# ZhenghaoFei/visual_odom

Hardware: AMD Instinct MI355X
Metric: stereo frames/sec on KITTI-00 1241x376 @ ~2000 features (higher is better)
Workload: dtype u8/int32 LK (f32 2x2 solve), f64 pose solve

## Files before the change

### visual_odom_amd/csrc/lk.hip

```cpp
#include "vo_kernels.h"
#include "vo_lkmath.h"

#include <float.h>
#include <type_traits>

namespace vo {

constexpr int LK_WIN = 21;
constexpr int LK_JT_W = 48, LK_JT_H = 40;
constexpr int LK_W_BITS = 14;
template <int W>
struct LkWin {
    static_assert(W % 2 == 1 && W >= 5 && W <= LK_WIN, "odd windows of 5 .. 21: the pyramid's borders are laid out for 21");
    static constexpr int SEGS = (W + 6) / 7, LANES = W * SEGS, COLS = 7 * SEGS + 1, ROWS = W + 1, LAST = W - 7 * (SEGS - 1);
    static constexpr int OFF_X = ((LK_JT_W - COLS) / 2) & ~3, OFF_Y = (LK_JT_H - ROWS) / 2;
    static_assert(LANES <= 64 && LK_JT_W >= COLS + OFF_X + 3 && LK_JT_H >= ROWS + OFF_Y, "the lane map and the tile hold the window");
};
constexpr uint32_t lk_seg_mask(int valid, int m)
{
    return (2 * m < valid ? 0x0000ffffu : 0u) | (2 * m + 1 < valid ? 0xffff0000u : 0u);
}

template <bool COLS>
__device__ __forceinline__ void lk_weights_packed(float a, float b, uint32_t &w0, uint32_t &w1)
{
    const float s = (float)(1 << LK_W_BITS), magic = 12582912.f;
    const float a1 = (1.f - a) * s, a0 = a * s, b1 = 1.f - b;
    const uint32_t r00 = (uint32_t)__float_as_int(a1 * b1 + magic);
    const uint32_t r01 = (uint32_t)__float_as_int(a0 * b1 + magic);
    const uint32_t r10 = (uint32_t)__float_as_int(a1 * b + magic);
    const uint32_t iw11 = ((1u << LK_W_BITS) + 3u * 0x4B400000u) - (r00 + r01 + r10);
    w0 = perm_b32(COLS ? r10 : r01, r00, VO_SEL_LO16);
    w1 = perm_b32(iw11, COLS ? r01 : r10, VO_SEL_LO16);
}
__device__ __forceinline__ void lk_weights(float a, float b, uint32_t &wt, uint32_t &wb)
{
    lk_weights_packed<false>(a, b, wt, wb);
}
__device__ __forceinline__ void lk_weights_cols(float a, float b, uint32_t &wl, uint32_t &wr)
{
    lk_weights_packed<true>(a, b, wl, wr);
}

struct LkOrigin {
    int x, y;
};
template <int W = LK_WIN>
__device__ __forceinline__ bool lk_tile_misses(bool have_tile, int jx0, int jy0, int inx, int iny)
{
    return !have_tile || inx < jx0 || inx + LkWin<W>::COLS > jx0 + LK_JT_W || iny < jy0 || iny + LkWin<W>::ROWS > jy0 + LK_JT_H;
}
template <int W = LK_WIN>
__device__ __forceinline__ LkOrigin lk_tile_origin(int jx_max, int jy_max, int inx, int iny)
{
    int jx0 = (inx - LkWin<W>::OFF_X) & ~3;
    int jy0 = iny - LkWin<W>::OFF_Y;
    jx0 = jx0 < -VO_BX ? -VO_BX : jx0 > jx_max ? jx_max : jx0;
    jy0 = jy0 < -VO_BY ? -VO_BY : jy0 > jy_max ? jy_max : jy0;
    return LkOrigin{jx0, jy0};
}
template <int W = LK_WIN>
__device__ __forceinline__ LkOrigin lk_tile_refill(uint8_t *tile, const VO_GLOBAL uint8_t *__restrict__ Jimg, int jstride, int jx_max, int jy_max,
                                               int inx, int iny, int c0, int step)
{
    const LkOrigin org = lk_tile_origin<W>(jx_max, jy_max, inx, iny);
    const int jx0 = org.x, jy0 = org.y;
    const VO_GLOBAL uint8_t *tb = Jimg + (ptrdiff_t)jy0 * jstride + jx0;
    for (int c = c0; c < LK_JT_H * (LK_JT_W / 16); c += step) {
        const int row = c / (LK_JT_W / 16), col = c - row * (LK_JT_W / 16);
        const U32x4A4 v = *(const VO_GLOBAL U32x4A4 *)(tb + (uint32_t)(row * jstride + 16 * col));
        *reinterpret_cast<uint4 *>(&tile[row * LK_JT_W + 16 * col]) = make_uint4(v.a, v.b, v.c, v.d);
    }
    return org;
}
template <int W = LK_WIN>
__device__ __forceinline__ LkOrigin lk_tile_refill_wave(uint8_t *tile, const VO_GLOBAL uint8_t *__restrict__ Jimg, int jstride, int jx_max,
                                                    int jy_max, int inx, int iny, int lane)
{
    constexpr int CPR = LK_JT_W / 16, CHUNKS = LK_JT_H * CPR;
    static_assert(CPR == 3 && CHUNKS > 64 && CHUNKS <= 128, "two chunks per lane at most; 64 chunks = 21 rows + 1 chunk");
    const LkOrigin org = lk_tile_origin<W>(jx_max, jy_max, inx, iny);
    const VO_GLOBAL uint8_t *tb = Jimg + (ptrdiff_t)org.y * jstride + org.x;
#ifndef VO_HOST_EMUL
    asm volatile("" : "+v"(lane));
#endif
    const int row = (lane * 43) >> 7, col = lane - CPR * row;
    const uint32_t g0 = (uint32_t)(row * jstride + 16 * col);
    const int next_col = 21 * jstride + 16, next_row = 22 * jstride - 16 * (CPR - 1);
    const uint32_t g1 = g0 + (uint32_t)(col == CPR - 1 ? next_row : next_col);
    const bool second = lane < CHUNKS - 64;
    const U32x4A4 v0 = *(const VO_GLOBAL U32x4A4 *)(tb + g0);
    U32x4A4 v1 = v0;
    if (second)
        v1 = *(const VO_GLOBAL U32x4A4 *)(tb + g1);
    *reinterpret_cast<uint4 *>(&tile[16 * lane]) = make_uint4(v0.a, v0.b, v0.c, v0.d);
    if (second)
        *reinterpret_cast<uint4 *>(&tile[16 * lane + 1024]) = make_uint4(v1.a, v1.b, v1.c, v1.d);
    return org;
}
template <int W = LK_WIN>
__device__ __forceinline__ LkOrigin lk_tile_cover(uint8_t *tile, const VO_GLOBAL uint8_t *__restrict__ Jimg, int jstride, int jx_max, int jy_max,
                                              int inx, int iny, int lane, bool have_tile, int jx0, int jy0)
{
    if (!lk_tile_misses<W>(have_tile, jx0, jy0, inx, iny))
        return LkOrigin{jx0, jy0};
    __syncthreads();
    const LkOrigin o = lk_tile_refill_wave<W>(tile, Jimg, jstride, jx_max, jy_max, inx, iny, lane);
    __syncthreads();
    return o;
}
__device__ __forceinline__ void lk_cell_rows(const uint8_t *tile, int off, uint32_t Jt[7], uint32_t Jb[7])
{
    const U32x2A1 t = *reinterpret_cast<const U32x2A1 *>(&tile[off]);
    const U32x2A1 u = *reinterpret_cast<const U32x2A1 *>(&tile[off + LK_JT_W]);
    lift7(t.a, t.b, Jt);
    lift7(u.a, u.b, Jb);
}
__device__ __forceinline__ void lk_cell_cols(const uint8_t *tile, int off, uint32_t Jc[8])
{
    const U32x2A1 t = *reinterpret_cast<const U32x2A1 *>(&tile[off]);
    const U32x2A1 u = *reinterpret_cast<const U32x2A1 *>(&tile[off + LK_JT_W]);
    lift8_cols(t.a, t.b, u.a, u.b, Jc);
}

#ifndef VO_LK_ATTRS
#define VO_LK_ATTRS __launch_bounds__(64, 7)
#endif
constexpr int VO_LK_USE_INITIAL_FLOW = 4, VO_LK_GET_MIN_EIGENVALS = 8;
template <bool SPLIT, bool ERR, int WIN = LK_WIN, bool FLAGS = false>
__device__ __forceinline__ void lk_circular_body(const PyrImage *__restrict__ imgs, const Quad *__restrict__ quads,
                                                 const float2 *__restrict__ pts_in, const int *__restrict__ n_pts, int cap,
                                                 int n_frames, int fpg , int ppp ,
                                                 float2 *__restrict__ trk,
                                                 uint8_t *__restrict__ status,
                                                 const LkParams prm, int hop_begin, int hop_end, float *__restrict__ err = nullptr,
                                                 int flags = 0)
{
    __shared__ __attribute__((aligned(16))) uint8_t s_jt[LK_JT_H * LK_JT_W];

    const int bid = blockIdx.x;
    const int xcd = bid & 7, slot = bid >> 3;
    const int grp = slot / ppp, fi = slot - grp * ppp;
    const int frame = grp * fpg + (xcd & (fpg - 1));
    const int f = (xcd / fpg) * ppp + fi;
    if (frame >= n_frames || f >= n_pts[frame])
        return;
    const int lane = threadIdx.x;
    using LW = LkWin<WIN>;
    const bool live = lane < LW::LANES;
    const int lr = live ? lane : LW::LANES - 1;
    const int r = lr / LW::SEGS, c0 = 7 * (lr - LW::SEGS * r);
    const int lane_off = r * LK_JT_W + c0;

    const Quad q = quads[frame];
    const float halfWin = (WIN - 1) * 0.5f;
    const float FLT_SCALE = 1.f / (1 << 20);
    const float eps_lo = (float)(prm.epsilon * 0.999999), eps_hi = (float)(prm.epsilon * 1.000001);
    const float min_eig_n = prm.min_eig * (1.001f * (float)(2 * WIN * WIN));

    const float2 p = pts_in[(size_t)frame * cap + f];
    float prevPtX = unif(p.x), prevPtY = unif(p.y);
    if (SPLIT && hop_begin > 0) {
        const size_t o = ((size_t)frame * 4 + (hop_begin - 1)) * cap + f;
        const float2 q0 = trk[o];
        const bool dead0 = status[o] == 0 || q0.x < 0.f || q0.y < 0.f || (hop_begin == 1 && (p.x < 0.f || p.y < 0.f));
        if (dead0 && !prm.full_chain)
            return;
        prevPtX = unif(q0.x);
        prevPtY = unif(q0.y);
    }

    for (int hop = SPLIT ? hop_begin : 0; hop < (ERR ? 1 : SPLIT ? hop_end : 4); hop++) {
        const int pi = hop == 0 ? q.l0 : hop == 1 ? q.r0 : hop == 2 ? q.r1 : q.l1;
        const int ni = hop == 0 ? q.r0 : hop == 1 ? q.r1 : hop == 2 ? q.l1 : q.l0;
        const PyrImage &I = imgs[pi];
        const PyrImage &J = imgs[ni];
        float outX = 0.f, outY = 0.f;
        int st = 1;
        float errv = 0.f;

        for (int level = prm.max_level; level >= 0; level--) {
            const float scale = __int_as_float((127 - level) << 23);
            float prevX = prevPtX * scale, prevY = prevPtY * scale;
            float nextX, nextY;
            if (level == prm.max_level) {
                nextX = prevX;
                nextY = prevY;
                if constexpr (FLAGS) {
                    if (flags & VO_LK_USE_INITIAL_FLOW) {
                        const float2 g = trk[(size_t)frame * cap + f];
                        nextX = unif(g.x) * scale;
                        nextY = unif(g.y) * scale;
                    }
                }
            } else {
                nextX = outX * 2.f;
                nextY = outY * 2.f;
            }
            outX = nextX;
            outY = nextY;

            const int iw = I.w[level], ih = I.h[level], istride = I.stride[level];
            const int jw = J.w[level], jh = J.h[level], jstride = J.stride[level];
            const VO_GLOBAL uint8_t *__restrict__ Iimg = (const VO_GLOBAL uint8_t *)I.lvl[level];
            const VO_GLOBAL uint32_t *__restrict__ Ider = (const VO_GLOBAL uint32_t *)I.der[level];
            const VO_GLOBAL uint8_t *__restrict__ Jimg = (const VO_GLOBAL uint8_t *)J.lvl[level];

            prevX -= halfWin;
            prevY -= halfWin;
            const float fpx = floorf(prevX), fpy = floorf(prevY);
            const int ipx = uni(vo_f2i(fpx)), ipy = uni(vo_f2i(fpy));
            if (VO_BALLOT(__builtin_isunordered(fpx, fpy)) != 0ull || ipx < -WIN || ipx >= iw || ipy < -WIN || ipy >= ih) {
                if (level == 0)
                    st = 0;
                continue;
            }
            uint32_t wl, wr;
            lk_weights_cols(prevX - fpx, prevY - fpy, wl, wr);

            uint32_t Ixp[4], Iyp[4];
            uint32_t Ipe[ERR ? 4 : 1];
            int a11 = 0, a12 = 0, a22 = 0, c1 = 0, c2 = 0;
            {
                const ptrdiff_t org = (ptrdiff_t)VO_BY * istride + VO_BX;
                const VO_GLOBAL uint8_t *Ib = Iimg - org;
                const VO_GLOBAL uint8_t *Db = (const VO_GLOBAL uint8_t *)(Ider - org);
                const uint32_t o = (uint32_t)((ipy + r + VO_BY) * istride + ipx + c0 + VO_BX);
                const uint32_t od = live ? 4u * o : 0u, drow = 4u * (uint32_t)istride;
                const U32x2A1 t = *(const VO_GLOBAL U32x2A1 *)(Ib + o);
                const U32x2A1 u = *(const VO_GLOBAL U32x2A1 *)(Ib + (o + (uint32_t)istride));
                const U32x4A4 dt0 = *(const VO_GLOBAL U32x4A4 *)(Db + od);
                const U32x4A4 dt1 = *(const VO_GLOBAL U32x4A4 *)(Db + (od + 16u));
                const U32x4A4 db0 = *(const VO_GLOBAL U32x4A4 *)(Db + (od + drow));
                const U32x4A4 db1 = *(const VO_GLOBAL U32x4A4 *)(Db + (od + drow + 16u));
                const uint32_t dt[8] = {dt0.a, dt0.b, dt0.c, dt0.d, dt1.a, dt1.b, dt1.c, dt1.d};
                const uint32_t db[8] = {db0.a, db0.b, db0.c, db0.d, db1.a, db1.b, db1.c, db1.d};
                uint32_t Ip[4];
                bilinear7_u8_cols(t.a, t.b, u.a, u.b, wl, wr, Ip);
                bilinear7_deriv_cols(dt, db, wl, wr, Ixp, Iyp);
                if constexpr (LW::LAST < 7) {
                    const bool part = LW::SEGS == 1 || c0 == 7 * (LW::SEGS - 1);
#pragma unroll
                    for (int m = 0; m < 4; m++) {
                        const uint32_t keep = part ? lk_seg_mask(LW::LAST, m) : 0xffffffffu;
                        Ixp[m] &= keep;
                        Iyp[m] &= keep;
                    }
                }
                a11 = sdot2_first(Ixp[0], Ixp[0], 0);
                a12 = sdot2_first(Ixp[0], Iyp[0], 0);
                a22 = sdot2_first(Iyp[0], Iyp[0], 0);
                c1 = sdot2_first(Ip[0], Ixp[0], 0);
                c2 = sdot2_first(Ip[0], Iyp[0], 0);
#pragma unroll
                for (int m = 1; m < 4; m++) {
                    a11 = sdot2(Ixp[m], Ixp[m], a11);
                    a12 = sdot2(Ixp[m], Iyp[m], a12);
                    a22 = sdot2(Iyp[m], Iyp[m], a22);
                    c1 = sdot2(Ip[m], Ixp[m], c1);
                    c2 = sdot2(Ip[m], Iyp[m], c2);
                }
                if constexpr (ERR) {
#pragma unroll
                    for (int m = 0; m < 4; m++)
                        Ipe[m] = Ip[m];
                }
            }
            float A11, A12, A22;
            wave_sum3_exact_f32(a11, a12, a22, A11, A12, A22);
            A11 *= FLT_SCALE;
            A12 *= FLT_SCALE;
            A22 *= FLT_SCALE;

            float D = A11 * A22 - A12 * A12;
            const float t = A22 + A11;
            const float s2 = (A11 - A22) * (A11 - A22) + 4.f * A12 * A12;
            const float u = t - (min_eig_n + t * 3.814697265625e-6f);
            bool eig_ok = u > 0.f && s2 < u * u * 0.9999f;
            if (__builtin_expect(!eig_ok, 0)) {
#ifndef VO_HOST_EMUL
                asm volatile("" ::: "memory");
#endif
                const float minEig = (t - sqrtf(s2)) / (float)(2 * WIN * WIN);
                eig_ok = !(minEig < prm.min_eig);
            }
            if constexpr (FLAGS) {
                if ((flags & VO_LK_GET_MIN_EIGENVALS) && level == 0)
                    errv = (t - sqrtf(s2)) / (float)(2 * WIN * WIN);
            }
            if (!eig_ok || D < FLT_EPSILON) {
                if (level == 0)
                    st = 0;
                continue;
            }
            D = 1.f / D;
            const float A11s = A11 * FLT_SCALE, A12s = A12 * FLT_SCALE, A22s = A22 * FLT_SCALE;
            const int nc1 = -c1, nc2 = -c2;

            nextX -= halfWin;
            nextY -= halfWin;
            float prevDX = 0.f, prevDY = 0.f;
            int jx0 = 0, jy0 = 0;
            bool have_tile = false;
            static_assert(LK_JT_W % 16 == 0 && VO_BX % 4 == 0, "16-byte tile chunks at 4-byte aligned origins");
            static_assert(VO_BY >= WIN && LK_JT_W >= LW::COLS + LW::OFF_X + 3 && LK_JT_H >= LW::ROWS + LW::OFF_Y,
                          "a tile clamped to the row end / the last border row still covers what the window of every corner the "
                          "reference admits reads (up to w - 1, h - 1: the borders are at least a window wide)");
            static_assert(VO_BY >= LW::COLS - 1, "right border (at least VO_BY columns) >= the columns a row reads beyond corner w - 1");
            const int jx_max = jstride - VO_BX - LK_JT_W, jy_max = jh + VO_BY - LK_JT_H;

            int j = 0;
            float fnx = floorf(nextX), fny = floorf(nextY);
            bool run = prm.max_count > 0;
            while (run) {
                const int inx = uni(vo_f2i(fnx)), iny = uni(vo_f2i(fny));
                if (VO_BALLOT(__builtin_isunordered(fnx, fny)) != 0ull || inx < -WIN || inx >= jw || iny < -WIN || iny >= jh) {
                    if (level == 0)
                        st = 0;
                    break;
                }
                {
                    const LkOrigin o = lk_tile_cover<WIN>(s_jt, Jimg, jstride, jx_max, jy_max, inx, iny, lane, have_tile, jx0, jy0);
                    jx0 = o.x;
                    jy0 = o.y;
                    have_tile = true;
                }
                uint32_t Jc[8];
                lk_cell_cols(s_jt, (iny - jy0) * LK_JT_W + (inx - jx0) + lane_off, Jc);
                for (;;) {
                    lk_weights_cols(nextX - fnx, nextY - fny, wl, wr);
                    int b1, b2;
                    {
                        uint32_t Jp[4];
                        blend7_cols(Jc, wl, wr, Jp);
                        b1 = sdot2_first(Jp[0], Ixp[0], nc1);
                        b2 = sdot2_first(Jp[0], Iyp[0], nc2);
#pragma unroll
                        for (int m = 1; m < 4; m++) {
                            b1 = sdot2(Jp[m], Ixp[m], b1);
                            b2 = sdot2(Jp[m], Iyp[m], b2);
                        }
                    }
                    float fb1, fb2;
                    wave_sum2_exact_f32(b1, b2, fb1, fb2);
                    const float dx = (A12s * fb2 - A22s * fb1) * D;
                    const float dy = (A12s * fb1 - A11s * fb2) * D;
                    nextX += dx;
                    nextY += dy;
                    outX = nextX + halfWin;
                    outY = nextY + halfWin;
                    const float n2 = fmaf(dy, dy, dx * dx);
                    if (__builtin_expect(!(n2 > eps_hi), 0)) {
#ifndef VO_HOST_EMUL
                        asm volatile("" ::: "memory");
#endif
                        if (n2 < eps_lo || (double)dx * dx + (double)dy * dy <= prm.epsilon) {
                            run = false;
                            break;
                        }
                    }
                    if (j > 0 && fabsf(dx + prevDX) <= 0.01f && fabsf(dy + prevDY) <= 0.01f) {
#ifndef VO_HOST_EMUL
                        asm volatile("" ::: "memory");
#endif
                        outX -= dx * 0.5f;
                        outY -= dy * 0.5f;
                        run = false;
                        break;
                    }
                    prevDX = dx;
                    prevDY = dy;
                    if (++j >= prm.max_count) {
                        run = false;
                        break;
                    }
                    const uint32_t ua = (uint32_t)__float_as_int(nextX - fnx), ub = (uint32_t)__float_as_int(nextY - fny);
                    if (VO_BALLOT((ua > ub ? ua : ub) >= 0x3f800000u) != 0ull) {
                        fnx = floorf(nextX);
                        fny = floorf(nextY);
                        break;
                    }
                }
            }

            if (st && level == 0 && (!FLAGS || !(flags & VO_LK_GET_MIN_EIGENVALS))) {
                const int fx = vo_f2i(floorf(outX - halfWin)), fy = vo_f2i(floorf(outY - halfWin));
                if (fx < -WIN || fx >= jw || fy < -WIN || fy >= jh)
                    st = 0;
                if constexpr (ERR) {
                    if (st && err != nullptr) {
                        const float ex = outX - halfWin, ey = outY - halfWin;
                        const float fex = floorf(ex), fey = floorf(ey);
                        const int inx = uni(fx), iny = uni(fy);
                        const LkOrigin o = lk_tile_cover<WIN>(s_jt, Jimg, jstride, jx_max, jy_max, inx, iny, lane, have_tile, jx0, jy0);
                        jx0 = o.x;
                        jy0 = o.y;
                        uint32_t Jc[8], Jp[4];
                        lk_cell_cols(s_jt, (iny - jy0) * LK_JT_W + (inx - jx0) + lane_off, Jc);
                        lk_weights_cols(ex - fex, ey - fey, wl, wr);
                        blend7_cols(Jc, wl, wr, Jp);
                        uint32_t e = 0;
#pragma unroll
                        for (int m = 0; m < 4; m++) {
                            if constexpr (LW::LAST < 7) {
                                const bool part = LW::SEGS == 1 || c0 == 7 * (LW::SEGS - 1);
                                e = udot2(pk_absdiff_i16(Jp[m], Ipe[m]) & (part ? lk_seg_mask(LW::LAST, m) : 0xffffffffu), 0x00010001u, e);
                            } else
                                e = udot2(pk_absdiff_i16(Jp[m], Ipe[m]), 0x00010001u, e);
                        }
                        errv = wave_sum_exact_f32(live ? (int)e : 0) / (float)(32 * WIN * WIN);
                    }
                }
            }
        }

        if constexpr (ERR) {
            if (lane == 0) {
                trk[(size_t)frame * cap + f] = make_float2(outX, outY);
                status[(size_t)frame * cap + f] = (uint8_t)st;
                if (err != nullptr) {
                    if constexpr (FLAGS)
                        err[(size_t)frame * cap + f] = ((flags & VO_LK_GET_MIN_EIGENVALS) || st) ? errv : 0.f;
                    else
                        err[(size_t)frame * cap + f] = st ? errv : 0.f;
                }
            }
            return;
        }
        if (lane == 0) {
            trk[((size_t)frame * 4 + hop) * cap + f] = make_float2(outX, outY);
            status[((size_t)frame * 4 + hop) * cap + f] = (uint8_t)st;
        }
        const bool dead = st == 0 || outX < 0.f || outY < 0.f || (hop == 0 && (p.x < 0.f || p.y < 0.f));
        if (dead && !prm.full_chain && hop < 3) {
            if (lane == 0)
                for (int k = hop + 1; k < 4; k++) {
                    trk[((size_t)frame * 4 + k) * cap + f] = make_float2(-1.f, -1.f);
                    status[((size_t)frame * 4 + k) * cap + f] = 0;
                }
            return;
        }
        prevPtX = unif(outX);
        prevPtY = unif(outY);
    }
}

__global__ VO_LK_ATTRS void lk_circular_kernel(const PyrImage *__restrict__ imgs,
                                                          const Quad *__restrict__ quads,
                                                          const float2 *__restrict__ pts_in,
                                                          const int *__restrict__ n_pts, int cap,
                                                          int n_frames, int fpg ,
                                                          int ppp ,
                                                          float2 *__restrict__ trk,
                                                          uint8_t *__restrict__ status,
                                                          LkParams prm)
{
    lk_circular_body<false, false>(imgs, quads, pts_in, n_pts, cap, n_frames, fpg, ppp, trk, status, prm, 0, 4);
}

__global__ VO_LK_ATTRS void lk_hops_kernel(const PyrImage *__restrict__ imgs, const Quad *__restrict__ quads,
                                           const float2 *__restrict__ pts_in, const int *__restrict__ n_pts, int cap,
                                           int n_frames, int fpg, int ppp, float2 *__restrict__ trk,
                                           uint8_t *__restrict__ status, LkParams prm, int hop_begin, int hop_end)
{
    lk_circular_body<true, false>(imgs, quads, pts_in, n_pts, cap, n_frames, fpg, ppp, trk, status, prm, hop_begin, hop_end);
}

#ifndef VO_LK_FLOW_ATTRS
#define VO_LK_FLOW_ATTRS __launch_bounds__(64, 6)
#endif
__global__ VO_LK_FLOW_ATTRS void lk_flow_kernel(const PyrImage *__restrict__ imgs, const Quad *__restrict__ pairs,
                                                const float2 *__restrict__ pts_in, const int *__restrict__ n_pts, int cap,
                                                int n_frames, int fpg, int ppp, float2 *__restrict__ next,
                                                uint8_t *__restrict__ status,
                                                float *__restrict__ err , LkParams prm)
{
    lk_circular_body<false, true>(imgs, pairs, pts_in, n_pts, cap, n_frames, fpg, ppp, next, status, prm, 0, 1, err);
}

template <int W>
__global__ VO_LK_FLOW_ATTRS void lk_flow_win_kernel(const PyrImage *__restrict__ imgs, const Quad *__restrict__ pairs,
                                                    const float2 *__restrict__ pts_in, const int *__restrict__ n_pts, int cap,
                                                    int n_frames, int fpg, int ppp, float2 *__restrict__ next,
                                                    uint8_t *__restrict__ status,
                                                    float *__restrict__ err , LkParams prm)
{
    static_assert(W < LK_WIN, "21 is lk_flow_kernel");
    lk_circular_body<false, true, W>(imgs, pairs, pts_in, n_pts, cap, n_frames, fpg, ppp, next, status, prm, 0, 1, err);
}

template <int W>
__global__ VO_LK_FLOW_ATTRS void lk_flow_flags_kernel(const PyrImage *__restrict__ imgs, const Quad *__restrict__ pairs,
                                                      const float2 *__restrict__ pts_in, const int *__restrict__ n_pts, int cap,
                                                      int n_frames, int fpg, int ppp, float2 *__restrict__ next,
                                                      uint8_t *__restrict__ status,
                                                      float *__restrict__ err , LkParams prm, int flags)
{
    lk_circular_body<false, true, W, true>(imgs, pairs, pts_in, n_pts, cap, n_frames, fpg, ppp, next, status, prm, 0, 1, err, flags);
}

struct LkGrid {
    int fpg, ppp, blocks;
};
inline LkGrid lk_grid(int n_frames, int n_items)
{
    const int fpg = n_frames >= 8 ? 8 : n_frames >= 4 ? 4 : n_frames >= 2 ? 2 : 1;
    const int parts = 8 / fpg, ppp = (n_items + parts - 1) / parts;
    const int groups = (n_frames + fpg - 1) / fpg;
    return {fpg, ppp, 8 * groups * ppp};
}

template <int... W, typename F>
inline bool lk_visit_window(int win, F &&f)
{
    return ((win == W && (f(std::integral_constant<int, W>{}), true)) || ...);
}
template <typename F>
inline bool lk_for_window(int win, F &&f)
{
    return lk_visit_window<5, 7, 9, 11, 13, 15, 17, 19, LK_WIN>(win, f);
}

template <int W, typename R>
inline void lk_flow_route(int flags, R &&run)
{
    if (flags != 0)
        run(lk_flow_flags_kernel<W>, flags);
    else if constexpr (W == LK_WIN)
        run(lk_flow_kernel);
    else
        run(lk_flow_win_kernel<W>);
}

#ifndef VO_HOST_EMUL
void launch_lk_flow(int win, int flags, const PyrImage *d_imgs, const Quad *d_pairs, const float2 *d_pts, const int *d_npts, int cap,
                    int max_pts, int n_frames, float2 *d_next, uint8_t *d_status, float *d_err, const LkParams &prm, hipStream_t stream)
{
    if (max_pts <= 0 || n_frames <= 0 || (flags & ~(VO_LK_USE_INITIAL_FLOW | VO_LK_GET_MIN_EIGENVALS)))
        return;
    const LkGrid g = lk_grid(n_frames, max_pts);
    lk_for_window(win, [&](auto w) {
        lk_flow_route<decltype(w)::value>(flags, [&](auto kernel, auto... tail) {
            hipLaunchKernelGGL(kernel, dim3((unsigned)g.blocks), dim3(64), 0, stream, d_imgs, d_pairs, d_pts, d_npts, cap, n_frames, g.fpg,
                               g.ppp, d_next, d_status, d_err, prm, tail...);
        });
    });
}

void launch_lk_circular(const PyrImage *d_imgs, const Quad *d_quads, const float2 *d_pts, const int *d_npts,
                        int cap, int max_pts, int n_frames, float2 *d_trk, uint8_t *d_status,
                        const LkParams &prm, hipStream_t stream)
{
    if (max_pts <= 0 || n_frames <= 0)
        return;
    const LkGrid g = lk_grid(n_frames, max_pts);
    hipLaunchKernelGGL(lk_circular_kernel, dim3((unsigned)g.blocks), dim3(64), 0, stream, d_imgs, d_quads, d_pts, d_npts, cap,
                       n_frames, g.fpg, g.ppp, d_trk, d_status, prm);
}

void launch_lk_hops(const PyrImage *d_imgs, const Quad *d_quads, const float2 *d_pts, const int *d_npts, int cap, int max_pts,
                    int n_frames, float2 *d_trk, uint8_t *d_status, const LkParams &prm, int hop_begin, int hop_end,
                    hipStream_t stream)
{
    if (max_pts <= 0 || n_frames <= 0 || hop_begin < 0 || hop_end > 4 || hop_begin >= hop_end)
        return;
    const LkGrid g = lk_grid(n_frames, max_pts);
    hipLaunchKernelGGL(lk_hops_kernel, dim3((unsigned)g.blocks), dim3(64), 0, stream, d_imgs, d_quads, d_pts, d_npts, cap, n_frames,
                       g.fpg, g.ppp, d_trk, d_status, prm, hop_begin, hop_end);
}

#endif

}

#ifdef VO_HOST_EMUL
#include "dev/lk_dev.hip"
#endif
```

### visual_odom_amd/csrc/vo_dev.h

```cpp
#pragma once

#include <stdint.h>

#ifdef VO_HOST_EMUL
#define VO_READFIRSTLANE(v) emu_readfirstlane(v)
#define VO_READLANE(v, l) emu_readlane((v), (l))
#define VO_UPDATE_DPP(old, src, ctrl, rm, bm, bc) emu_update_dpp((old), (src), (ctrl), (rm), (bm), (bc))
#define VO_BALLOT(p) emu_ballot(p)
#define VO_POPCLL(m) __builtin_popcountll(m)
#define VO_MBCNT(m, acc, lane) ((acc) + (uint32_t)__builtin_popcountll((m) & ((1ull << (lane)) - 1ull)))
#define VO_PERMLANE32_SWAP(a, b) emu_permlane_swap((a), (b), 32)
#define VO_PERMLANE16_SWAP(a, b) emu_permlane_swap((a), (b), 16)
#else
#include <hip/hip_runtime.h>
#define VO_READFIRSTLANE(v) __builtin_amdgcn_readfirstlane(v)
#define VO_READLANE(v, l) __builtin_amdgcn_readlane((v), (l))
#define VO_UPDATE_DPP(old, src, ctrl, rm, bm, bc) __builtin_amdgcn_update_dpp((old), (src), (ctrl), (rm), (bm), (bc))
#define VO_BALLOT(p) __builtin_amdgcn_ballot_w64(p)
#define VO_POPCLL(m) __popcll(m)
#define VO_MBCNT(m, acc, lane) __builtin_amdgcn_mbcnt_hi((uint32_t)((m) >> 32), __builtin_amdgcn_mbcnt_lo((uint32_t)(m), (acc)))
#define VO_PERMLANE32_SWAP(a, b)                                                                      \
    do {                                                                                              \
        auto r_ = __builtin_amdgcn_permlane32_swap((unsigned)(a), (unsigned)(b), false, false);       \
        (a) = (int)r_[0];                                                                             \
        (b) = (int)r_[1];                                                                             \
    } while (0)
#define VO_PERMLANE16_SWAP(a, b)                                                                      \
    do {                                                                                              \
        auto r_ = __builtin_amdgcn_permlane16_swap((unsigned)(a), (unsigned)(b), false, false);       \
        (a) = (int)r_[0];                                                                             \
        (b) = (int)r_[1];                                                                             \
    } while (0)
#endif

#if defined(__HIP_DEVICE_COMPILE__) && !defined(VO_HOST_EMUL)
#define VO_GLOBAL __attribute__((address_space(1)))
#else
#define VO_GLOBAL
#endif

#define VO_MAX_LEVELS 5
#define VO_BX 32
#define VO_BY 24
static_assert(VO_BX % 16 == 0 && VO_BX >= 21 && VO_BY >= 21, "pixel (0, 0) of a row is 16-byte aligned; 21 x 21 windows at -21 read border, not the neighbour row");

namespace vo {

struct PyrImage {
    uint8_t *lvl[VO_MAX_LEVELS];
    uint32_t *der[VO_MAX_LEVELS];
    int w[VO_MAX_LEVELS], h[VO_MAX_LEVELS], stride[VO_MAX_LEVELS];
};

struct Quad {
    int l0, r0, l1, r1;
};

struct __attribute__((packed, aligned(1))) U32x2A1 {
    uint32_t a, b;
};
struct __attribute__((packed, aligned(2))) U32x2A2 {
    uint32_t a, b;
};
struct __attribute__((packed, aligned(1))) U32x4A1 {
    uint32_t a, b, c, d;
};
struct __attribute__((packed, aligned(4))) U32x4A4 {
    uint32_t a, b, c, d;
};

__device__ __forceinline__ int reflect101(int p, int len)
{
    if (len == 1)
        return 0;
    while (p < 0 || p >= len)
        p = p < 0 ? -p : 2 * (len - 1) - p;
    return p;
}

__device__ __forceinline__ int vo_f2i(float v)
{
#ifdef VO_HOST_EMUL
    if (v != v)
        return 0;
    if (v >= 2147483648.f)
        return 2147483647;
    if (v <= -2147483648.f)
        return -2147483647 - 1;
#endif
    return (int)v;
}
__device__ __forceinline__ int vo_d2i(double v)
{
#ifdef VO_HOST_EMUL
    if (v != v)
        return 0;
    if (v >= 2147483647.0)
        return 2147483647;
    if (v <= -2147483648.0)
        return -2147483647 - 1;
#endif
    return (int)v;
}

__device__ __forceinline__ int uni(int v) { return VO_READFIRSTLANE(v); }
__device__ __forceinline__ float unif(float v)
{
    return __int_as_float(VO_READFIRSTLANE(__float_as_int(v)));
}

#define VO_DPP_QUAD_XOR1 0xB1
#define VO_DPP_QUAD_XOR2 0x4E
#define VO_DPP_ROW_HALF_MIRROR 0x141
#define VO_DPP_ROW_MIRROR 0x140
#define VO_DPP_ROW_BCAST15 0x142
#define VO_DPP_ROW_BCAST31 0x143

template <int CTRL, int ROW_MASK>
__device__ __forceinline__ int dpp_add(int v)
{
    return v + VO_UPDATE_DPP(0, v, CTRL, ROW_MASK, 0xf, true);
}

__device__ __forceinline__ float wave_sum_exact_f32(int v)
{
    v = dpp_add<VO_DPP_QUAD_XOR1, 0xf>(v);
    v = dpp_add<VO_DPP_QUAD_XOR2, 0xf>(v);
    v = dpp_add<VO_DPP_ROW_HALF_MIRROR, 0xf>(v);
    int lo = v & 0xffff, hi = v >> 16;
    lo = dpp_add<VO_DPP_ROW_MIRROR, 0xf>(lo);
    hi = dpp_add<VO_DPP_ROW_MIRROR, 0xf>(hi);
    lo = dpp_add<VO_DPP_ROW_BCAST15, 0xa>(lo);
    hi = dpp_add<VO_DPP_ROW_BCAST15, 0xa>(hi);
    lo = dpp_add<VO_DPP_ROW_BCAST31, 0xc>(lo);
    hi = dpp_add<VO_DPP_ROW_BCAST31, 0xc>(hi);
    return fmaf((float)VO_READLANE(hi, 63), 65536.f, (float)VO_READLANE(lo, 63));
}

__device__ __forceinline__ void wave_sum2_exact_f32(int a, int b, float &fa, float &fb)
{
    VO_PERMLANE32_SWAP(a, b);
    int t = a + b;
    t = dpp_add<VO_DPP_QUAD_XOR1, 0xf>(t);
    t = dpp_add<VO_DPP_QUAD_XOR2, 0xf>(t);
    int hi = t >> 16, lo = t & 0xffff;
    VO_PERMLANE16_SWAP(hi, lo);
    int u = hi + lo;
    u = dpp_add<VO_DPP_ROW_HALF_MIRROR, 0xf>(u);
    u = dpp_add<VO_DPP_ROW_MIRROR, 0xf>(u);
    const float uf = (float)u;
    const float up = __int_as_float(VO_UPDATE_DPP(0, __float_as_int(uf), VO_DPP_ROW_BCAST15, 0xa, 0xf, true));
    const float res = fmaf(up, 65536.f, uf);
    fa = __int_as_float(VO_READLANE(__float_as_int(res), 31));
    fb = __int_as_float(VO_READLANE(__float_as_int(res), 63));
}

__device__ __forceinline__ void wave_sum3_exact_f32(int a, int b, int c, float &fa, float &fb, float &fc)
{
    int z = 0;
    VO_PERMLANE32_SWAP(a, b);
    int t1 = a + b;
    VO_PERMLANE32_SWAP(c, z);
    int t2 = c + z;
    VO_PERMLANE16_SWAP(t1, t2);
    int u = t1 + t2;
    u = dpp_add<VO_DPP_QUAD_XOR1, 0xf>(u);
    int hi = u >> 16, lo = u & 0xffff;
    hi = dpp_add<VO_DPP_QUAD_XOR2, 0xf>(hi);
    lo = dpp_add<VO_DPP_QUAD_XOR2, 0xf>(lo);
    hi = dpp_add<VO_DPP_ROW_HALF_MIRROR, 0xf>(hi);
    lo = dpp_add<VO_DPP_ROW_HALF_MIRROR, 0xf>(lo);
    hi = dpp_add<VO_DPP_ROW_MIRROR, 0xf>(hi);
    lo = dpp_add<VO_DPP_ROW_MIRROR, 0xf>(lo);
    const float r = fmaf((float)hi, 65536.f, (float)lo);
    fa = __int_as_float(VO_READLANE(__float_as_int(r), 0));
    fc = __int_as_float(VO_READLANE(__float_as_int(r), 16));
    fb = __int_as_float(VO_READLANE(__float_as_int(r), 32));
}

}
```

Before: 23460.

## Flatten LK iteration loop, unroll by two, and pack bilinear weight math

Replaces the nested per-cell/per-iteration LK loop with one flat loop unrolled by two. The previous displacement ping-pongs between two register pairs, so the per-iteration copy disappears. The cell-exit check and cell reload are folded into the iteration, and the output position plus oscillation correction are computed once after exit instead of every step. It also computes the bilinear weight products as a two-wide float vector with fma scaling, and passes the DPP old operand as the live value instead of zero to save a move. The gain relies on the compiler actually emitting fewer moves and branches. The restructured exit codes add complexity and risk subtle behaviour differences.

```diff
diff --git a/visual_odom_amd/csrc/lk.hip b/visual_odom_amd/csrc/lk.hip
--- a/visual_odom_amd/csrc/lk.hip
+++ b/visual_odom_amd/csrc/lk.hip
@@ -25,10 +25,12 @@
 __device__ __forceinline__ void lk_weights_packed(float a, float b, uint32_t &w0, uint32_t &w1)
 {
     const float s = (float)(1 << LK_W_BITS), magic = 12582912.f;
-    const float a1 = (1.f - a) * s, a0 = a * s, b1 = 1.f - b;
-    const uint32_t r00 = (uint32_t)__float_as_int(a1 * b1 + magic);
-    const uint32_t r01 = (uint32_t)__float_as_int(a0 * b1 + magic);
-    const uint32_t r10 = (uint32_t)__float_as_int(a1 * b + magic);
+    typedef float F32x2 __attribute__((vector_size(8)));
+    const F32x2 p = {a, b}, q = 1.f - p, pswap = {b, a};
+    const F32x2 x = q * pswap;
+    const uint32_t r00 = (uint32_t)__float_as_int(fmaf(q[0] * q[1], s, magic));
+    const uint32_t r01 = (uint32_t)__float_as_int(fmaf(x[1], s, magic));
+    const uint32_t r10 = (uint32_t)__float_as_int(fmaf(x[0], s, magic));
     const uint32_t iw11 = ((1u << LK_W_BITS) + 3u * 0x4B400000u) - (r00 + r01 + r10);
     w0 = perm_b32(COLS ? r10 : r01, r00, VO_SEL_LO16);
     w1 = perm_b32(iw11, COLS ? r01 : r10, VO_SEL_LO16);
@@ -299,7 +301,6 @@
 
             nextX -= halfWin;
             nextY -= halfWin;
-            float prevDX = 0.f, prevDY = 0.f;
             int jx0 = 0, jy0 = 0;
             bool have_tile = false;
             static_assert(LK_JT_W % 16 == 0 && VO_BX % 4 == 0, "16-byte tile chunks at 4-byte aligned origins");
@@ -310,76 +311,109 @@
             const int jx_max = jstride - VO_BX - LK_JT_W, jy_max = jh + VO_BY - LK_JT_H;
 
             int j = 0;
-            float fnx = floorf(nextX), fny = floorf(nextY);
-            bool run = prm.max_count > 0;
-            while (run) {
-                const int inx = uni(vo_f2i(fnx)), iny = uni(vo_f2i(fny));
-                if (VO_BALLOT(__builtin_isunordered(fnx, fny)) != 0ull || inx < -WIN || inx >= jw || iny < -WIN || iny >= jh) {
-                    if (level == 0)
-                        st = 0;
-                    break;
-                }
+            int left = 0;
+            float fnx = 0.f, fny = 0.f, frx = 0.f, fry = 0.f;
+            uint32_t J0, J1, J2, J3, J4, J5, J6, J7;
+#ifndef VO_HOST_EMUL
+            asm volatile("" : "=v"(J0), "=v"(J1), "=v"(J2), "=v"(J3), "=v"(J4), "=v"(J5), "=v"(J6), "=v"(J7));
+#else
+            J0 = J1 = J2 = J3 = J4 = J5 = J6 = J7 = 0;
+#endif
+            int inx = 0, iny = 0;
+            bool cell = true;
+            auto cell_admitted = [&]() -> bool {
+                fnx = floorf(nextX);
+                fny = floorf(nextY);
+                inx = uni(vo_f2i(fnx));
+                iny = uni(vo_f2i(fny));
+                return !(VO_BALLOT(__builtin_isunordered(fnx, fny)) != 0ull || inx < -WIN || inx >= jw || iny < -WIN || iny >= jh);
+            };
+            auto enter_cell = [&]() {
                 {
                     const LkOrigin o = lk_tile_cover<WIN>(s_jt, Jimg, jstride, jx_max, jy_max, inx, iny, lane, have_tile, jx0, jy0);
                     jx0 = o.x;
                     jy0 = o.y;
                     have_tile = true;
                 }
-                uint32_t Jc[8];
-                lk_cell_cols(s_jt, (iny - jy0) * LK_JT_W + (inx - jx0) + lane_off, Jc);
+                uint32_t Jn[8];
+                lk_cell_cols(s_jt, (iny - jy0) * LK_JT_W + (inx - jx0) + lane_off, Jn);
+                J0 = Jn[0], J1 = Jn[1], J2 = Jn[2], J3 = Jn[3], J4 = Jn[4], J5 = Jn[5], J6 = Jn[6], J7 = Jn[7];
+                frx = nextX - fnx;
+                fry = nextY - fny;
+            };
+            auto iterate = [&](const float px, const float py, float &dx, float &dy, const int osc) -> int {
+                lk_weights_cols(frx, fry, wl, wr);
+                int b1, b2;
+                {
+                    const uint32_t Jc[8] = {J0, J1, J2, J3, J4, J5, J6, J7};
+                    uint32_t Jp[4];
+                    blend7_cols(Jc, wl, wr, Jp);
+                    b1 = sdot2_first(Jp[0], Ixp[0], nc1);
+                    b2 = sdot2_first(Jp[0], Iyp[0], nc2);
+#pragma unroll
+                    for (int m = 1; m < 4; m++) {
+                        b1 = sdot2(Jp[m], Ixp[m], b1);
+                        b2 = sdot2(Jp[m], Iyp[m], b2);
+                    }
+                }
+                float fb1, fb2;
+                wave_sum2_exact_f32(b1, b2, fb1, fb2);
+                dx = (A12s * fb2 - A22s * fb1) * D;
+                dy = (A12s * fb1 - A11s * fb2) * D;
+                nextX += dx;
+                nextY += dy;
+                const float n2 = fmaf(dy, dy, dx * dx);
+                if (__builtin_expect(!(n2 > eps_hi), 0)) {
+#ifndef VO_HOST_EMUL
+                    asm volatile("" ::: "memory");
+#endif
+                    if (n2 < eps_lo || (double)dx * dx + (double)dy * dy <= prm.epsilon)
+                        return 1;
+                }
+                if (j > 0 && fabsf(dx + px) <= 0.01f && fabsf(dy + py) <= 0.01f)
+                    return osc;
+                if (++j >= prm.max_count)
+                    return 1;
+                frx = nextX - fnx;
+                fry = nextY - fny;
+                const uint32_t ua = (uint32_t)__float_as_int(frx), ub = (uint32_t)__float_as_int(fry);
+                cell = VO_BALLOT((ua > ub ? ua : ub) >= 0x3f800000u) != 0ull;
+                if (cell && !cell_admitted())
+                    return 4;
+                return 0;
+            };
+            float dAx = 0.f, dAy = 0.f, dBx = 0.f, dBy = 0.f;
+            bool run = prm.max_count > 0;
+            if (run && !cell_admitted()) {
+                if (level == 0)
+                    st = 0;
+                run = false;
+            }
+            if (run)
                 for (;;) {
-                    lk_weights_cols(nextX - fnx, nextY - fny, wl, wr);
-                    int b1, b2;
-                    {
-                        uint32_t Jp[4];
-                        blend7_cols(Jc, wl, wr, Jp);
-                        b1 = sdot2_first(Jp[0], Ixp[0], nc1);
-                        b2 = sdot2_first(Jp[0], Iyp[0], nc2);
-#pragma unroll
-                        for (int m = 1; m < 4; m++) {
-                            b1 = sdot2(Jp[m], Ixp[m], b1);
-                            b2 = sdot2(Jp[m], Iyp[m], b2);
-                        }
-                    }
-                    float fb1, fb2;
-                    wave_sum2_exact_f32(b1, b2, fb1, fb2);
-                    const float dx = (A12s * fb2 - A22s * fb1) * D;
-                    const float dy = (A12s * fb1 - A11s * fb2) * D;
-                    nextX += dx;
-                    nextY += dy;
-                    outX = nextX + halfWin;
-                    outY = nextY + halfWin;
-                    const float n2 = fmaf(dy, dy, dx * dx);
-                    if (__builtin_expect(!(n2 > eps_hi), 0)) {
+                    if (cell)
+                        enter_cell();
+                    if ((left = iterate(dBx, dBy, dAx, dAy, 2)) != 0)
+                        break;
+                    if (cell)
+                        enter_cell();
+                    if ((left = iterate(dAx, dAy, dBx, dBy, 3)) != 0)
+                        break;
+                }
+            if (left == 4 && level == 0)
+                st = 0;
+            if (left != 0) {
 #ifndef VO_HOST_EMUL
-                        asm volatile("" ::: "memory");
-#endif
-                        if (n2 < eps_lo || (double)dx * dx + (double)dy * dy <= prm.epsilon) {
-                            run = false;
-                            break;
-                        }
-                    }
-                    if (j > 0 && fabsf(dx + prevDX) <= 0.01f && fabsf(dy + prevDY) <= 0.01f) {
+                asm volatile("" ::: "memory");
+#endif
+                outX = nextX + halfWin;
+                outY = nextY + halfWin;
+                if (left == 2 || left == 3) {
 #ifndef VO_HOST_EMUL
-                        asm volatile("" ::: "memory");
-#endif
-                        outX -= dx * 0.5f;
-                        outY -= dy * 0.5f;
-                        run = false;
-                        break;
-                    }
-                    prevDX = dx;
-                    prevDY = dy;
-                    if (++j >= prm.max_count) {
-                        run = false;
-                        break;
-                    }
-                    const uint32_t ua = (uint32_t)__float_as_int(nextX - fnx), ub = (uint32_t)__float_as_int(nextY - fny);
-                    if (VO_BALLOT((ua > ub ? ua : ub) >= 0x3f800000u) != 0ull) {
-                        fnx = floorf(nextX);
-                        fny = floorf(nextY);
-                        break;
-                    }
+                    asm volatile("" ::: "memory");
+#endif
+                    outX -= (left == 2 ? dAx : dBx) * 0.5f;
+                    outY -= (left == 2 ? dAy : dBy) * 0.5f;
                 }
             }
 
diff --git a/visual_odom_amd/csrc/vo_dev.h b/visual_odom_amd/csrc/vo_dev.h
--- a/visual_odom_amd/csrc/vo_dev.h
+++ b/visual_odom_amd/csrc/vo_dev.h
@@ -149,7 +149,7 @@
     u = dpp_add<VO_DPP_ROW_HALF_MIRROR, 0xf>(u);
     u = dpp_add<VO_DPP_ROW_MIRROR, 0xf>(u);
     const float uf = (float)u;
-    const float up = __int_as_float(VO_UPDATE_DPP(0, __float_as_int(uf), VO_DPP_ROW_BCAST15, 0xa, 0xf, true));
+    const float up = __int_as_float(VO_UPDATE_DPP(u, __float_as_int(uf), VO_DPP_ROW_BCAST15, 0xa, 0xf, true));
     const float res = fmaf(up, 65536.f, uf);
     fa = __int_as_float(VO_READLANE(__float_as_int(res), 31));
     fb = __int_as_float(VO_READLANE(__float_as_int(res), 63));
```

Result: faster. 24440, median of 6 (+4.1%).
